# MoseleyBioinformaticsLab/ICIKendallTau

Hardware: AMD Instinct MI355X
Metric: column-pairs/s (+ full-matrix wall time) at 10k feat x 1k samp (higher is better)
Workload: dtype int32 rank/popcount counting + f64 epilogue

## Files before the change

icikendalltau_amd/csrc/icikt_capi.cpp:

```cpp
#include <hip/hip_runtime.h>

#include <algorithm>
#include <chrono>
#include <cstdio>
#include <cstring>
#include <functional>
#include <new>
#include <string>
#include <vector>

#include "icikt.h"
#include "icikt_device.h"
#include "icikt_host.h"

using icikt::ColStats;
using icikt::PairRaw;
using icikt::PrepView;

static_assert(ICIKT_CNT_FIELDS == icikt::ICIKT_CNT_FIELDS_, "counts record layout");
static_assert(ICIKT_PERSPECTIVE_LOCAL == icikt::ICIKT_PERSPECTIVE_LOCAL_, "perspective code");

namespace {

int flush_timer(icikt_ctx* c, int k) {
// ... 1486 lines not shown
                                      d_dst, dst_ld, c->d_csc_err.p, c->stream));
  unsigned long long rec[icikt::ICIKT_CSC_ERR_WORDS] = {};
  HIPCHK(c, hipMemcpyAsync(rec, c->d_csc_err.p, sizeof(rec), hipMemcpyDeviceToHost, c->stream));
  HIPCHK(c, hipStreamSynchronize(c->stream));
  if (rec[0] != 0) return fail(c, ICIKT_E_INVALID, "scatter_csc: " + icikt::host::csc_message(rec));
  return ICIKT_SUCCESS;
}

}

extern "C" {

int icikt_debug_set_plan(icikt_ctx* c, const char* spec) {
  if (!c) return ICIKT_E_INVALID;
  icikt_ctx::PlanOverride ov;
  int pipe = -1, k0 = -1;
  std::string sp = spec ? spec : "";
  size_t pos = 0;
  while (pos < sp.size()) {
    size_t end = sp.find(',', pos);
    if (end == std::string::npos) end = sp.size();
    const std::string item = sp.substr(pos, end - pos);
    pos = end + 1;
    if (item.empty()) continue;
    const size_t eq = item.find('=');
    if (eq == std::string::npos) return fail(c, ICIKT_E_INVALID, "debug_set_plan: expected key=value, got '" + item + "'");
    const std::string key = item.substr(0, eq), val = item.substr(eq + 1);
    if (val.empty()) continue;
    if (key == "np") ov.np = atoi(val.c_str());
    else if (key == "pend") ov.pend = (val[0] == 'g') ? 1 : 0;
    else if (key == "wpb") ov.wpb = atoi(val.c_str());
    else if (key == "half") ov.half = (val[0] == '1') ? 1 : 0;
    else if (key == "hyb") ov.hyb = (val[0] == '1') ? 1 : 0;
    else if (key == "tgmax") { ov.has_tgmax = true; ov.tgmax = atoi(val.c_str()); }
    else if (key == "list") ov.list = atoi(val.c_str());
    else if (key == "solo") ov.solo = atoi(val.c_str());
    else if (key == "split") ov.split = atoi(val.c_str());
    else if (key == "merge") ov.merge = atoi(val.c_str());
    else if (key == "waves") ov.waves = atoi(val.c_str());
    else if (key == "verbose") ov.verbose = (val[0] == '1');
    else if (key == "gridmult") ov.grid_mult = atoi(val.c_str());
    else if (key == "gridcap") ov.grid_cap = atoi(val.c_str());
    else if (key == "pipe") pipe = (val[0] == '1') ? 1 : 0;
    else if (key == "k0") k0 = (val[0] == '1') ? 1 : 0;
    else if (key == "tkblock") ov.tkblock = atoll(val.c_str());
    else if (key == "medlds") {
      ov.medlds = atoi(val.c_str());
      if (ov.medlds < 0 || ov.medlds > icikt::MEDIAN_STAGE_MAX)
        return fail(c, ICIKT_E_INVALID, "debug_set_plan: medlds must be in 0 .. 4096 keys");
    }
    else if (key == "qbatch") {
      ov.qbatch = atoi(val.c_str());
      if (ov.qbatch < 1 || ov.qbatch > icikt::QUANT_BATCH_MAX)
        return fail(c, ICIKT_E_INVALID, "debug_set_plan: qbatch must be in 1 .. 32 targets");
    }
    else return fail(c, ICIKT_E_INVALID, "debug_set_plan: unknown key '" + key + "'");
  }
  c->plan_ov = ov;
  c->pipe_mode = pipe;
  c->k0_shape = k0;

  c->raw_valid = false;
  c->wpb = 0;
  return ICIKT_SUCCESS;
}

int icikt_debug_step_stats(icikt_ctx* c, uint64_t* out24, int reset) {
  if (!c || !out24) return ICIKT_E_INVALID;
  int rc = use_device(c);
  if (rc) return rc;
  HIPCHK(c, hipStreamSynchronize(c->stream));
  unsigned long long tmp[24];
  const hipError_t e = icikt::read_step_stats(tmp, reset);
  if (e == hipErrorNotSupported) { (void)hipGetLastError(); return fail(c, ICIKT_E_STATE, "debug_step_stats: not a -DICIKT_STEP_STATS build"); }
  HIPCHK(c, e);
  for (int i = 0; i < 24; ++i) out24[i] = tmp[i];
  return ICIKT_SUCCESS;
}

int icikt_selftest(icikt_ctx* c) {
  if (!c) return ICIKT_E_INVALID;
  int rc = use_device(c);
  if (rc) return rc;
  HIPCHK(c, c->d_self.reserve(640));
  HIPCHK(c, icikt::launch_selftest(c->d_self.p, c->stream));
  uint32_t h[640];
  HIPCHK(c, hipMemcpyAsync(h, c->d_self.p, sizeof(h), hipMemcpyDeviceToHost, c->stream));
  HIPCHK(c, hipStreamSynchronize(c->stream));
  for (uint32_t l = 0; l < 64; ++l) {
    if (h[l] != (l + 1) * (l + 2) / 2) return fail(c, ICIKT_E_HIP, "selftest: wave_incl_scan mismatch");
    if (h[64 + l] != (l == 0 ? 0xABCDu : 3u * (l - 1))) return fail(c, ICIKT_E_HIP, "selftest: wave_shr1 mismatch");
    if (h[128 + l] != (l < 41 ? 0xFFFFFFFFu : l - 41)) return fail(c, ICIKT_E_HIP, "selftest: repeated wave_shr1 mismatch");
    if (h[256 + l] != (l < 32 ? l : 100u + (l - 32))) return fail(c, ICIKT_E_HIP, "selftest: permlane32_swap[0] mismatch");
    if (h[320 + l] != (l < 32 ? 32u + l : 100u + l)) return fail(c, ICIKT_E_HIP, "selftest: permlane32_swap[1] mismatch");
    const uint32_t k = (l & 31u) + 1, b = (l & 32u) + 1;
    if (h[384 + l] != k * (2 * b + k - 1) / 2) return fail(c, ICIKT_E_HIP, "selftest: half_incl_scan mismatch");
    if (h[448 + l] != 63u) {
      if (c->plan_ov.verbose) fprintf(stderr, "[icikt] selftest lane %u: lane_xor pass mask %u\n", l, h[448 + l]);
      return fail(c, ICIKT_E_HIP, "selftest: lane_xor mismatch");
    }
  }
  for (uint32_t half = 0; half < 2; ++half) {
    uint32_t want = 0, got = 0;
    for (uint32_t l = half * 32; l < half * 32 + 32; ++l) {
      const uint32_t lo = ((l * 40503u + 977u) >> 3) & 0xFFFu;
      for (uint32_t j = half * 32; j < l; ++j) want += (((j * 2654435761u >> 20) & 0xFFFu) < lo) ? 1u : 0u;
      got += h[192 + l];
    }
    if (got != want) {
      if (c->plan_ov.verbose) fprintf(stderr, "[icikt] selftest half %u: got %u want %u\n", half, got, want);
      return fail(c, ICIKT_E_HIP, "selftest: half_allpairs mismatch");
    }
  }
  for (uint32_t half = 0; half < 2; ++half) {
    uint32_t want = 0, got = 0;
    for (uint32_t l = half * 32; l < half * 32 + 32; ++l) {
      const uint32_t lo = ((l * 40503u + 977u) >> 3) & 0xFFFu, lo2 = ((l * 69069u + 12345u) >> 5) & 0x27BFu;
      for (uint32_t j = half * 32; j < l; ++j) {
        want += (((j * 2654435761u >> 20) & 0xFFFu) < lo) ? 1u : 0u;
        want += (((j * 1103515245u >> 17) & 0x27BFu) < lo2) ? 1u : 0u;
      }
      got += h[576 + l];
    }
    if (got != want) {
      if (c->plan_ov.verbose) fprintf(stderr, "[icikt] selftest half %u (packed): got %u want %u\n", half, got, want);
      return fail(c, ICIKT_E_HIP, "selftest: half_step_count mismatch");
    }
  }
  return ICIKT_SUCCESS;
}

}
```

icikendalltau_amd/csrc/icikt_kernels.hip:

```cpp
#include <hip/hip_runtime.h>
#include <stdint.h>
#include <stdlib.h>

#include <algorithm>
#include <type_traits>

#include "icikt_device.h"
#include "icikt_wave.h"

namespace icikt {

struct WaveLds {
  unsigned long long* seen;
  uint16_t* spre;
};

#define ICIKT_HSHR(b) "v_sub_co_u32_dpp %1, vcc, %2, %3 row_shr:" #b " row_mask:0xf bank_mask:0xf bound_ctrl:0\n\t" \
                      "v_addc_co_u32_e32 %0, vcc, 0, %0, vcc\n\t"
#define ICIKT_HROR(b) "v_sub_co_u32_dpp %1, vcc, %4, %5 row_ror:" #b " row_mask:0xf bank_mask:0xf\n\t" \
                      "v_addc_co_u32_e32 %0, vcc, 0, %0, vcc\n\t"
__device__ __forceinline__ uint32_t half_allpairs(uint32_t q, uint32_t lo, uint32_t xa, uint32_t xb, uint32_t lane) {
  uint32_t acc = 0, junk;
  asm volatile("s_nop 1\n\t"
               ICIKT_HSHR(1) ICIKT_HSHR(2) ICIKT_HSHR(3) ICIKT_HSHR(4) ICIKT_HSHR(5) ICIKT_HSHR(6) ICIKT_HSHR(7)
// ... 13 lines not shown
  const uint32_t rot = (uint32_t)__builtin_amdgcn_update_dpp(0, (int)r[1], 0x121 , 0xf, 0xf, false);
  const uint32_t xa = (lane & 16u) ? r[0] : rot;
  return half_allpairs(q, lo, xa, ~offer, lane);
}

#define ICIKT_PACC  "v_perm_b32 %1, %1, %2, %6\n\tv_lshrrev_b32_e32 %0, 1, %0\n\tv_and_or_b32 %0, %1, %5, %0\n\t"
#define ICIKT_PSHR2(a, b) "v_add_u32_dpp %1, %3, %4 row_shr:" #a " row_mask:0xf bank_mask:0xf bound_ctrl:0\n\t" \
                          "v_add_u32_dpp %2, %3, %4 row_shr:" #b " row_mask:0xf bank_mask:0xf bound_ctrl:0\n\t" ICIKT_PACC
#define ICIKT_PROR2(a, b) "v_add_u32_dpp %1, %3, %4 row_ror:" #a " row_mask:0xf bank_mask:0xf\n\t" \
                          "v_add_u32_dpp %2, %3, %4 row_ror:" #b " row_mask:0xf bank_mask:0xf\n\t" ICIKT_PACC
__device__ __forceinline__ uint32_t half_partner_addr(uint32_t lane) {
  const uint32_t p = lane & 15u, h = lane & 32u;
  return ((lane & 16u) ? (h + p) : (h + 16u + ((p + 15u) & 15u))) * 4u;
}
struct HalfChain { uint32_t A, B, offer, xa; };
__device__ __forceinline__ HalfChain half_step_prep(uint32_t sw0, uint32_t sw1, uint32_t lane, uint32_t partner_addr) {
  HalfChain h;
  const uint32_t Q = __builtin_amdgcn_perm(sw1, sw0, 0x05040100u);
  const uint32_t LO = __builtin_amdgcn_perm(sw1, sw0, 0x07060302u);
  h.A = 0x7FFF7FFFu - Q; h.B = LO;
  h.offer = (lane & 16u) ? h.B : h.A;
  h.xa = (uint32_t)__builtin_amdgcn_ds_bpermute((int)partner_addr, (int)h.offer);
  return h;
}
__device__ __forceinline__ uint32_t half_step_part_a(const HalfChain& h, uint32_t acc) {
  const uint32_t A = h.A, B = h.B, xa = h.xa, offer = h.offer;
  const uint32_t M8 = 0x80808080u, SEL = 0x07050301u;
  uint32_t v1, t1, t2;
  asm volatile("s_nop 1\n\t"
               "v_add_u32_dpp %1, %3, %4 row_shr:1 row_mask:0xf bank_mask:0xf bound_ctrl:0\n\t"
               "v_add_u32_dpp %2, %3, %4 row_shr:2 row_mask:0xf bank_mask:0xf bound_ctrl:0\n\t"
               "v_perm_b32 %1, %1, %2, %6\n\tv_and_b32_e32 %0, %5, %1\n\t"
               ICIKT_PSHR2(3, 4) ICIKT_PSHR2(5, 6) ICIKT_PSHR2(7, 8) ICIKT_PSHR2(9, 10) ICIKT_PSHR2(11, 12)
               ICIKT_PSHR2(13, 14)
               "v_add_u32_dpp %1, %3, %4 row_shr:15 row_mask:0xf bank_mask:0xf bound_ctrl:0\n\t"
               "v_add_u32_e32 %2, %7, %8\n\t" ICIKT_PACC
               : "=&v"(v1), "=&v"(t1), "=&v"(t2)
               : "v"(A), "v"(B), "s"(M8), "s"(SEL), "v"(xa), "v"(offer));
  return bcnt_acc(v1, acc);
}
__device__ __forceinline__ uint32_t half_step_part_b(const HalfChain& h, uint32_t acc) {
  const uint32_t xa = h.xa, offer = h.offer;
  const uint32_t M8 = 0x80808080u, SEL = 0x07050301u, M16 = 0x80008000u;
  uint32_t v2, t1, t2;
  asm volatile("s_nop 1\n\t"
               "v_add_u32_dpp %1, %3, %4 row_ror:1 row_mask:0xf bank_mask:0xf\n\t"
               "v_add_u32_dpp %2, %3, %4 row_ror:2 row_mask:0xf bank_mask:0xf\n\t"
               "v_perm_b32 %1, %1, %2, %6\n\tv_and_b32_e32 %0, %5, %1\n\t"
               ICIKT_PROR2(3, 4) ICIKT_PROR2(5, 6)
               "v_add_u32_dpp %1, %3, %4 row_ror:7 row_mask:0xf bank_mask:0xf\n\t"
               "v_lshrrev_b32_e32 %0, 1, %0\n\tv_and_or_b32 %0, %1, %7, %0\n\t"
               : "=&v"(v2), "=&v"(t1), "=&v"(t2)
               : "v"(xa), "v"(offer), "s"(M8), "s"(SEL), "s"(M16));
  return bcnt_acc(v2, acc);
}
__device__ __forceinline__ uint32_t half_step_count(uint32_t sw0, uint32_t sw1, uint32_t lane, uint32_t partner_addr) {
  const uint32_t Q = __builtin_amdgcn_perm(sw1, sw0, 0x05040100u);
  const uint32_t LO = __builtin_amdgcn_perm(sw1, sw0, 0x07060302u);
  const uint32_t A = 0x7FFF7FFFu - Q, B = LO;
  const uint32_t offer = (lane & 16u) ? B : A;
  const uint32_t xa = (uint32_t)__builtin_amdgcn_ds_bpermute((int)partner_addr, (int)offer);
  const uint32_t M8 = 0x80808080u, SEL = 0x07050301u, M16 = 0x80008000u;
  uint32_t v1, v2, t1, t2;
  asm volatile("s_nop 1\n\t"
               "v_add_u32_dpp %1, %3, %4 row_shr:1 row_mask:0xf bank_mask:0xf bound_ctrl:0\n\t"
               "v_add_u32_dpp %2, %3, %4 row_shr:2 row_mask:0xf bank_mask:0xf bound_ctrl:0\n\t"
               "v_perm_b32 %1, %1, %2, %6\n\tv_and_b32_e32 %0, %5, %1\n\t"
               ICIKT_PSHR2(3, 4) ICIKT_PSHR2(5, 6) ICIKT_PSHR2(7, 8) ICIKT_PSHR2(9, 10) ICIKT_PSHR2(11, 12)
               ICIKT_PSHR2(13, 14)
               "v_add_u32_dpp %1, %3, %4 row_shr:15 row_mask:0xf bank_mask:0xf bound_ctrl:0\n\t"
               "v_add_u32_e32 %2, %7, %8\n\t" ICIKT_PACC
               : "=&v"(v1), "=&v"(t1), "=&v"(t2)
               : "v"(A), "v"(B), "s"(M8), "s"(SEL), "v"(xa), "v"(offer));
  asm volatile("s_nop 1\n\t"
               "v_add_u32_dpp %1, %3, %4 row_ror:1 row_mask:0xf bank_mask:0xf\n\t"
               "v_add_u32_dpp %2, %3, %4 row_ror:2 row_mask:0xf bank_mask:0xf\n\t"
               "v_perm_b32 %1, %1, %2, %6\n\tv_and_b32_e32 %0, %5, %1\n\t"
               ICIKT_PROR2(3, 4) ICIKT_PROR2(5, 6)
               "v_add_u32_dpp %1, %3, %4 row_ror:7 row_mask:0xf bank_mask:0xf\n\t"
               "v_lshrrev_b32_e32 %0, 1, %0\n\tv_and_or_b32 %0, %1, %7, %0\n\t"
               : "=&v"(v2), "=&v"(t1), "=&v"(t2)
               : "v"(xa), "v"(offer), "s"(M8), "s"(SEL), "s"(M16));
  return bcnt_acc(v2, bcnt_acc(v1, 0u));
}

__device__ __forceinline__ void half_step_flags(uint32_t src, uint32_t own, uint32_t offer, uint32_t partner_addr,
                                                uint32_t& v1, uint32_t& v2) {
  const uint32_t xa = (uint32_t)__builtin_amdgcn_ds_bpermute((int)partner_addr, (int)offer);
  const uint32_t M8 = 0x80808080u, SEL = 0x07050301u, M16 = 0x80008000u;
  uint32_t t1, t2;
  asm volatile("s_nop 1\n\t"
               "v_add_u32_dpp %1, %3, %4 row_shr:1 row_mask:0xf bank_mask:0xf bound_ctrl:0\n\t"
               "v_add_u32_dpp %2, %3, %4 row_shr:2 row_mask:0xf bank_mask:0xf bound_ctrl:0\n\t"
               "v_perm_b32 %1, %1, %2, %6\n\tv_and_b32_e32 %0, %5, %1\n\t"
               ICIKT_PSHR2(3, 4) ICIKT_PSHR2(5, 6) ICIKT_PSHR2(7, 8) ICIKT_PSHR2(9, 10) ICIKT_PSHR2(11, 12)
               ICIKT_PSHR2(13, 14)
               "v_add_u32_dpp %1, %3, %4 row_shr:15 row_mask:0xf bank_mask:0xf bound_ctrl:0\n\t"
               "v_add_u32_e32 %2, %7, %8\n\t" ICIKT_PACC
               : "=&v"(v1), "=&v"(t1), "=&v"(t2)
               : "v"(src), "v"(own), "s"(M8), "s"(SEL), "v"(xa), "v"(offer));
  asm volatile("s_nop 1\n\t"
               "v_add_u32_dpp %1, %3, %4 row_ror:1 row_mask:0xf bank_mask:0xf\n\t"
               "v_add_u32_dpp %2, %3, %4 row_ror:2 row_mask:0xf bank_mask:0xf\n\t"
               "v_perm_b32 %1, %1, %2, %6\n\tv_and_b32_e32 %0, %5, %1\n\t"
               ICIKT_PROR2(3, 4) ICIKT_PROR2(5, 6)
               "v_add_u32_dpp %1, %3, %4 row_ror:7 row_mask:0xf bank_mask:0xf\n\t"
               "v_lshrrev_b32_e32 %0, 1, %0\n\tv_and_or_b32 %0, %1, %7, %0\n\t"
               : "=&v"(v2), "=&v"(t1), "=&v"(t2)
               : "v"(xa), "v"(offer), "s"(M8), "s"(SEL), "s"(M16));
}

template <int C>
__device__ __forceinline__ void half_step_flags_near(uint32_t src, uint32_t own, uint32_t offer, uint32_t partner_addr,
                                                     uint32_t& v1, uint32_t& v2) {
  const uint32_t xa = (uint32_t)__builtin_amdgcn_ds_bpermute((int)partner_addr, (int)offer);
  const uint32_t M8 = 0x80808080u, SEL = 0x07050301u, M16 = 0x80008000u;
  uint32_t t1, t2;
#define ICIKT_NEAR_HEAD "s_nop 1\n\t"                                                                          \
               "v_add_u32_dpp %1, %3, %4 row_shr:1 row_mask:0xf bank_mask:0xf bound_ctrl:0\n\t"                \
               "v_add_u32_dpp %2, %3, %4 row_shr:2 row_mask:0xf bank_mask:0xf bound_ctrl:0\n\t"                \
               "v_perm_b32 %1, %1, %2, %6\n\tv_and_b32_e32 %0, %5, %1\n\t"
  if constexpr (C == 0) {
    asm volatile(ICIKT_NEAR_HEAD "v_lshrrev_b32_e32 %0, 7, %0\n\t"
                 : "=&v"(v1), "=&v"(t1), "=&v"(t2) : "v"(src), "v"(own), "s"(M8), "s"(SEL));
  } else if constexpr (C == 1) {
    asm volatile(ICIKT_NEAR_HEAD ICIKT_PSHR2(3, 4) "v_lshrrev_b32_e32 %0, 6, %0\n\t"
                 : "=&v"(v1), "=&v"(t1), "=&v"(t2) : "v"(src), "v"(own), "s"(M8), "s"(SEL));
  } else {
    asm volatile(ICIKT_NEAR_HEAD ICIKT_PSHR2(3, 4) ICIKT_PSHR2(5, 6) ICIKT_PSHR2(7, 8) "v_lshrrev_b32_e32 %0, 4, %0\n\t"
                 : "=&v"(v1), "=&v"(t1), "=&v"(t2) : "v"(src), "v"(own), "s"(M8), "s"(SEL));
  }
#undef ICIKT_NEAR_HEAD
#define ICIKT_NEAR_HEAD2 "s_nop 1\n\t"                                                                         \
               "v_add_u32_dpp %1, %3, %4 row_ror:1 row_mask:0xf bank_mask:0xf\n\t"                             \
               "v_add_u32_dpp %2, %3, %4 row_ror:2 row_mask:0xf bank_mask:0xf\n\t"                             \
               "v_perm_b32 %1, %1, %2, %6\n\tv_and_b32_e32 %0, %5, %1\n\t"
  if constexpr (C == 0) {
    asm volatile(ICIKT_NEAR_HEAD2 "v_lshrrev_b32_e32 %0, 3, %0\n\t"
                 : "=&v"(v2), "=&v"(t1), "=&v"(t2) : "v"(xa), "v"(offer), "s"(M8), "s"(SEL));
  } else if constexpr (C == 1) {
    asm volatile(ICIKT_NEAR_HEAD2 ICIKT_PROR2(3, 4) "v_lshrrev_b32_e32 %0, 2, %0\n\t"
                 : "=&v"(v2), "=&v"(t1), "=&v"(t2) : "v"(xa), "v"(offer), "s"(M8), "s"(SEL));
  } else {
    asm volatile(ICIKT_NEAR_HEAD2 ICIKT_PROR2(3, 4) ICIKT_PROR2(5, 6)
                 "v_add_u32_dpp %1, %3, %4 row_ror:7 row_mask:0xf bank_mask:0xf\n\t"
                 "v_lshrrev_b32_e32 %0, 1, %0\n\tv_and_or_b32 %0, %1, %7, %0\n\t"
                 : "=&v"(v2), "=&v"(t1), "=&v"(t2) : "v"(xa), "v"(offer), "s"(M8), "s"(SEL), "s"(M16));
  }
#undef ICIKT_NEAR_HEAD2
}

__device__ __forceinline__ uint32_t wave_cross_idx(uint32_t lane, uint32_t c) {
  const uint32_t later = (c == 1u) ? (lane & 16u) : (lane & 32u);
  const uint32_t prow = (lane ^ (c << 4)) & 48u;
  return (prow | ((later ? lane : lane - 1u) & 15u)) << 2;
}
#define ICIKT_WROR(b, xa, xb) "v_sub_co_u32_dpp %1, vcc, " xa ", " xb " row_ror:" #b " row_mask:0xf bank_mask:0xf\n\t" \
                              "v_addc_co_u32_e32 %0, vcc, 0, %0, vcc\n\t"
#define ICIKT_WROUND(xa, xb)                                                                  \
  "v_cmp_lt_u32_e32 vcc, " xa ", " xb "\n\tv_addc_co_u32_e32 %0, vcc, 0, %0, vcc\n\t"        \
  ICIKT_WROR(1, xa, xb) ICIKT_WROR(2, xa, xb) ICIKT_WROR(3, xa, xb) ICIKT_WROR(4, xa, xb)     \
  ICIKT_WROR(5, xa, xb) ICIKT_WROR(6, xa, xb) ICIKT_WROR(7, xa, xb)
__device__ __forceinline__ uint32_t wave_allpairs(uint32_t q, uint32_t lo, uint32_t lane) {
  const uint32_t nlo = ~lo;
  const uint32_t off1 = (lane & 16u) ? nlo : q;
  const uint32_t off2 = (lane & 32u) ? nlo : q;
// ... 343 lines not shown
    my_ctr = task_ctr + xg;
    int t = 0;
    if (lane == 0u) t = atomicAdd(my_ctr, 1);
    task = t_lo + __builtin_amdgcn_readfirstlane(t);
  }
  const int split = half_mode_of<NP, HI>() ? k1_opt_segments(opts) : 1;
  int seg = 0;
  if (split > 1) {
    seg = gwave / n_tasks;
    task = gwave - seg * n_tasks;
    if (seg >= split) return;
  }
  if (task >= t_hi) return;
  do {
  ICIKT_ST_DECL
  int pidx[NP];
  pidx[0] = __builtin_amdgcn_readfirstlane(tasks[2 * task]);
  const int p_second = __builtin_amdgcn_readfirstlane(tasks[2 * task + 1]);
  const int np = (NP == 2 && p_second >= 0) ? 2 : 1;
  if (NP == 2) pidx[NP - 1] = (p_second >= 0) ? p_second : pidx[0];

  const int scol = __builtin_amdgcn_readfirstlane(pj[pidx[0]]);
  const uint16_t* ord = pv.order + (int64_t)scol * pv.n_ord;
  const uint32_t* ord_w = pv.order_w ? pv.order_w + (int64_t)scol * pv.n_ord : nullptr;
  const unsigned long long* gf = pv.col_gflag(scol);
  const unsigned long long* ma = pv.col_mask(scol);
  const unsigned long long* fa = pv.col_fillmask(scol);

  uint32_t comp[NP];
  const uint16_t* hiG[NP];
  const uint32_t* tgB[NP];
  int ntgB[NP];
  bool cntB[NP];
  PairState S[NP];
  uint32_t cb[NP], gg[NP];
  bool g_oddtie = false;
  const uint32_t* rec_blk;
  const uint32_t* hi_blk;
  const uint32_t* gi_blk;
  {
    const int g0 = __builtin_amdgcn_readfirstlane(pi[pidx[0]]);
    rec_blk = pv.rec + ((int64_t)(g0 >> 1) * pv.rec_rows) * 2;
    hi_blk = reinterpret_cast<const uint32_t*>(pv.hirow + ((int64_t)(g0 >> 1) * pv.rec_rows) * 2);
    gi_blk = reinterpret_cast<const uint32_t*>(pv.girow + ((int64_t)(g0 >> 1) * pv.rec_rows) * 2);
  }
#pragma unroll
  for (int k = 0; k < NP; ++k) {
    const int gcol = __builtin_amdgcn_readfirstlane(pi[pidx[k]]);
    comp[k] = (uint32_t)(gcol & 1);
    hiG[k] = pv.hirow + ((int64_t)(gcol >> 1) * pv.rec_rows) * 2 + (gcol & 1);
    tgB[k] = pv.tgroups + (int64_t)gcol * pv.tg_stride;
    const int ntg_raw = __builtin_amdgcn_readfirstlane((int)pv.col_stats(gcol)->ntg);
    cntB[k] = half_mode ? (ntg_raw > tg_list) : (ntg_raw > max(tg_list, K1_CNT_MIN_GROUPS));
    ntgB[k] = (!(opts & K1_OPT_ROW_ONLY) && ntg_raw <= ((half_mode || cntB[k]) ? max(tg_list, tg_max) : tg_list)) ? ntg_raw : -1;
    g_oddtie = g_oddtie || (__builtin_amdgcn_readfirstlane(pv.col_stats(gcol)->flags) & COL_ODD_TIE) != 0;
    const unsigned long long* mb = pv.col_mask(gcol);
    const unsigned long long* fb = pv.col_fillmask(gcol);

    unsigned char* wbase = smem + ((size_t)wave * NP + k) * (size_t)perpair_bytes;
    S[k].L.seen = reinterpret_cast<unsigned long long*>(wbase);
    if (HI == 0) {
      S[k].L.spre = reinterpret_cast<uint16_t*>(S[k].L.seen + Wp4);
      for (int w = lane; w < Wp4; w += 64) S[k].L.seen[w] = 0ull;
      uint32_t* tl32 = reinterpret_cast<uint32_t*>(S[k].L.spre);
      for (int w = lane; w < (TL_BYTES + (cnt_cap > 0 ? (cnt_cap + 2) * ICIKT_CNT_BYTES + 3 : 0)) / 4; w += 64) tl32[w] = 0u;
    } else {
      S[k].L.spre = reinterpret_cast<uint16_t*>(S[k].L.seen + Wp4);
      for (int w = lane; w < Wp4; w += 64) S[k].L.seen[w] = 0ull;
      for (int w = lane; w < k1_half_pre_bytes<(HI > 0 ? HI : 1)>() / 2; w += 64) S[k].L.spre[w] = 0;
      uint32_t* cz = reinterpret_cast<uint32_t*>(reinterpret_cast<unsigned char*>(S[k].L.spre) + k1_half_pre_bytes<(HI > 0 ? HI : 1)>());
      for (int w = lane; w < ((tg_max + 2) * ICIKT_CNT_BYTES + 3) / 4; w += 64) cz[w] = 0u;
    }
    S[k].dis = 0; S[k].tie = 0; S[k].tie2 = 0;
    cb[k] = 0; gg[k] = 0;
    if (seg == 0) {
      for (int w = lane; w < W; w += 64) {
        cb[k] += (uint32_t)__popcll(ma[w] & mb[w]);
        gg[k] += (uint32_t)__popcll(fa[w] & fb[w]);
      }
    }
  }
  wave_lds_fence();

  uint32_t r0 = gload_u16(ord, lane), r1 = gload_u16(ord, 64u + lane), r2 = gload_u16(ord, 128u + lane);
  uint32_t rk_pre[NP];
  uint2 rv_pre = make_uint2(0u, 0u);
  bool rk_ok = false;
#pragma unroll
  for (int k = 0; k < NP; ++k) rk_pre[k] = 0u;
  uint32_t hi_pre = 0;
  uint32_t gi_pre = 0;
  bool hi_ok = false;

  const uint32_t solo_cap = (uint32_t)max(0, (tg_max + 1) * ICIKT_CNT_BYTES);
  bool solo_ok = half_mode && !(opts & K1_OPT_ROW_ONLY) && !(opts & K1_OPT_NO_SOLO);
#pragma unroll
  for (int k = 0; k < NP; ++k) solo_ok = solo_ok && (pv.col_stats(__builtin_amdgcn_readfirstlane(pi[pidx[k]]))->ntg <= solo_cap);
  int last_start;
  bool closed_form = true;
#pragma unroll
  for (int k = 0; k < NP; ++k) closed_form = closed_form && (ntgB[k] >= 0);
  int hot_until;
  {
    int best = 0, first_cont = n;
    for (int w = lane; w < W; w += 64) {
      unsigned long long f = gf[w];
      unsigned long long z = ~f;
      if (w == W - 1 && (n & 63)) { f &= (1ull << (n & 63)) - 1ull; z &= (1ull << (n & 63)) - 1ull; }
      if (f != 0ull) best = max(best, w * 64 + 63 - (int)__builtin_clzll(f));
      if (z != 0ull) first_cont = min(first_cont, w * 64 + (int)__builtin_ctzll(z));
    }
    last_start = __builtin_amdgcn_readfirstlane(wave_max_i32(best));
    first_cont = -__builtin_amdgcn_readfirstlane(wave_max_i32(-first_cont));
    hot_until = (first_cont < n) ? first_cont - 1 : n;
    closed_form = closed_form && (n - last_start > 64);
  }
  int seg_begin = 0, seg_end = n, seg_step = -1;
  if constexpr (half_mode) {
    if (split > 1) {
      const uint32_t* tail = pv.tprog + (int64_t)scol * pv.tp_stride + (pv.tp_stride - 2 * TPROG_MARKS);
      const uint32_t mv = gload_u32(tail, lane & 7u);
      auto mark = [&](int j, int& mp, int& ms) {
        mp = (int)min((uint32_t)__builtin_amdgcn_readlane((int)mv, j), (uint32_t)n);
        ms = __builtin_amdgcn_readlane((int)mv, 4 + j);
      };
      int b1 = n, b2 = n, b3 = n, s1 = -1, s2 = -1, s3 = -1;
      if (split == 2) mark(1, b1, s1);
      else { mark(0, b1, s1); mark(2, b2, s2); mark(3, b3, s3); }
      seg_begin = (seg == 0) ? 0 : (seg == 1) ? b1 : (seg == 2) ? b2 : b3;
      seg_end = (seg == 0) ? b1 : (seg == 1) ? b2 : (seg == 2) ? b3 : n;
      seg_step = (seg == 0) ? -1 : (seg == 1) ? s1 : (seg == 2) ? s2 : s3;
      if (seg > 0 && seg_begin >= seg_end) return;
      closed_form = closed_form && (seg_end >= n);
      hot_until = min(hot_until, seg_end);
    }
  }
  const int end_main = min(closed_form ? last_start : n, seg_end);

  const uint32_t partner_addr = half_partner_addr(lane);
  uint32_t dis_half = 0, dis_half_neg = 0;
  uint32_t seg_tie = 0, seg_tie2 = 0;
  bool grp_open = false;
  int grp_start = 0, grp_entries = 0;
  uint32_t sv_k0 = 0, sv_k1 = 0, sv_h = 0;
  uint32_t sv_kw[NP], sv_hw[NP], sv_gw[NP], sneg[NP];
#pragma unroll
  for (int k = 0; k < NP; ++k) { sv_kw[k] = 0u; sv_hw[k] = 0u; sv_gw[k] = 0u; sneg[k] = 0u; }
  int pos = 0;
  if constexpr (half_mode) {
    if (seg_begin > 0) {
      constexpr int HP = (HI > 0 ? HI : 1);
      const bool hiP = lane >= 32u;
      const uint32_t l32p = lane & 31u;
      unsigned long long* seenP = hiP ? S[NP - 1].L.seen : S[0].L.seen;
      uint16_t* spreP = hiP ? S[NP - 1].L.spre : S[0].L.spre;
      const uint32_t GUARDP = (uint32_t)W << 6;
      const uint32_t ord_last = (uint32_t)pv.n_ord - 1u;
      uint32_t rw[4];
#pragma unroll
      for (int u = 0; u < 4; ++u) rw[u] = gload_u16(ord, min((uint32_t)u * 64u + lane, ord_last));
      for (int p = 0; p < seg_begin; p += 256) {
        uint2 rv[4];
#pragma unroll
        for (int u = 0; u < 4; ++u) rv[u] = gload_rec2(rec_blk, rw[u]);
#pragma unroll
        for (int u = 0; u < 4; ++u) rw[u] = gload_u16(ord, min((uint32_t)p + 256u + (uint32_t)u * 64u + lane, ord_last));
#pragma unroll
        for (int u = 0; u < 4; ++u) {
          const int pu = p + 64 * u;
          const auto sw = __builtin_amdgcn_permlane32_swap(comp[0] ? rv[u].y : rv[u].x, comp[NP - 1] ? rv[u].y : rv[u].x, false, false);
          const bool w0 = pu + (int)l32p < seg_begin, w1 = pu + 32 + (int)l32p < seg_begin;
          seen_insert(seenP, w0 ? (sw[0] & 0xFFFFu) : GUARDP);
          seen_insert(seenP, w1 ? (sw[1] & 0xFFFFu) : GUARDP);
        }
      }
      wave_lds_fence();
      rebuild_prefix_half<HP>(seenP, spreP, l32p);
      wave_lds_fence();
      pos = seg_begin;
      r0 = gload_u16(ord, (uint32_t)pos + lane);
      r1 = gload_u16(ord, (uint32_t)pos + 64u + lane);
      r2 = gload_u16(ord, (uint32_t)pos + 128u + lane);
    }
  }
  ICIKT_ST_MARK(6, 0)
  unsigned long long fw0 = 0ull, fw1 = 0ull;
  int fw_word = -1;
  const uint32_t* tprog_col = half_mode ? pv.tprog + (int64_t)scol * pv.tp_stride : nullptr;
  const uint16_t* srow_col = half_mode ? pv.srow + (int64_t)scol * pv.sr_steps * 64 : nullptr;
  const uint2* smask_col = half_mode ? pv.smask + (int64_t)scol * pv.sr_steps * 32 : nullptr;
  uint32_t tp_a = 0u, tp_b = 0u;
  int tp_step = 0;
  bool tp_ok = false;
  auto advance64 = [&]() {
    r0 = r1; r1 = r2;
    if (NP == 2) rv_pre = gload_rec2(rec_blk, r0);
    else rk_pre[0] = gload_u32(rec_blk, 2u * r0 + comp[0]);
    r2 = gload_u16(ord, (uint32_t)pos + 128u + lane);
    rk_ok = true;
  };
  auto take_rk = [&](uint32_t (&rk)[NP]) {
    if (NP == 2) {
#pragma unroll
      for (int k = 0; k < NP; ++k) rk[k] = comp[k] ? rv_pre.y : rv_pre.x;
    } else {
      rk[0] = rk_pre[0];
    }
  };
  bool defer_allpairs = false;
  uint32_t mix_sg1 = 0u, mix_sg2 = 0u;
  int mix_cls = 3;
  uint32_t solo_g0 = 0u, solo_g1 = 0u;
  auto hot_step = [&](const uint32_t (&rk)[NP], auto mode_tag) {
    constexpr int MODE = decltype(mode_tag)::value;
    constexpr bool MIXED = MODE == 1;
    if constexpr (half_mode) {
      const auto sw = __builtin_amdgcn_permlane32_swap(rk[0], rk[NP - 1], false, false);
      const bool hi = lane >= 32u;
      unsigned long long* seenH = hi ? S[NP - 1].L.seen : S[0].L.seen;
      uint16_t* spreH = hi ? S[NP - 1].L.spre : S[0].L.spre;
      const uint32_t l32 = lane & 31u;
      constexpr int H = (HI > 0 ? HI : 1);
      uint32_t inpairs = 0;
#pragma unroll
      for (int sub = 0; sub < 2; ++sub) {
        const uint32_t r = sub ? sw[1] : sw[0];
        const uint32_t qh = r & 0xFFFFu, loh = r >> 16;
        const uint32_t wlo = r >> 22;
        const uint32_t dlo = (wlo * (65536u / (uint32_t)H + 1u)) >> 16;
        const uint32_t pre_lo = (uint32_t)*reinterpret_cast<const uint16_t*>(
            reinterpret_cast<const unsigned char*>(spreH) + 2u * wlo + (2u * (uint32_t)k1_half_slot<H>() - 2u * (uint32_t)H) * dlo);
        const unsigned long long word_lo = seenH[wlo];
        wave_lds_fence();
        atomicOr(reinterpret_cast<uint32_t*>(seenH) + __builtin_amdgcn_ubfe(r, 5, 10), 1u << (qh & 31u));
        wave_lds_fence();
        unsigned long long wv[H];
#pragma unroll
        for (int i = 0; i < H; ++i) wv[i] = seenH[l32 * (uint32_t)H + (uint32_t)i];
        uint32_t solo_c = 1u;
        uint8_t* cntS = nullptr;
        if constexpr (MODE == 2) {
          const uint32_t g = sub ? solo_g1 : solo_g0;
          cntS = reinterpret_cast<uint8_t*>(spreH) + k1_half_pre_bytes<H>();
          if (g < solo_cap) atomicAdd(reinterpret_cast<uint32_t*>(cntS) + (g >> 2), 1u << ((g & 3u) << 3));
          wave_lds_fence();
          solo_c = (g < solo_cap) ? (uint32_t)cntS[g] : 1u;
        }
        if (sub == 0 && MODE != 2) {
          if constexpr (!MIXED) {
            inpairs = half_step_count(sw[0], sw[1], lane, partner_addr);
          } else {
            const uint32_t Q = __builtin_amdgcn_perm(sw[1], sw[0], 0x05040100u);
            const uint32_t LO = __builtin_amdgcn_perm(sw[1], sw[0], 0x07060302u);
            const uint32_t A = 0x7FFF7FFFu - Q, B = LO;
            uint32_t f1, f2, g1, g2;
            half_step_flags(A, B, (lane & 16u) ? B : A, partner_addr, f1, f2);
            if (mix_cls == 0) half_step_flags_near<0>(B, A, (lane & 16u) ? A : B, partner_addr, g1, g2);
            else if (mix_cls == 1) half_step_flags_near<1>(B, A, (lane & 16u) ? A : B, partner_addr, g1, g2);
            else if (mix_cls == 2) half_step_flags_near<2>(B, A, (lane & 16u) ? A : B, partner_addr, g1, g2);
            else half_step_flags(B, A, (lane & 16u) ? A : B, partner_addr, g1, g2);
            inpairs = bcnt_acc(f2 & ~mix_sg2, bcnt_acc(f1 & ~mix_sg1, 0u));
            seg_tie = bcnt_acc(mix_sg2 & ~(f2 | g2), bcnt_acc(mix_sg1 & ~(f1 | g1), seg_tie));
          }
        }
        uint32_t pre_lo_k = pre_lo;
        unsigned long long word_lo_k = word_lo;
        asm volatile("" : "+v"(pre_lo_k), "+v"(word_lo_k));
#pragma unroll
        for (int i = 0; i < H; ++i) asm volatile("" : "+v"(wv[i]));
        dis_half += pre_lo_k + (sub == 0 ? inpairs : 0u);
        dis_half_neg = bcnt64_acc(word_lo_k >> (loh & 63u), dis_half_neg);
        uint32_t cw[H], run = 0;
#pragma unroll
        for (int i = 0; i < H; ++i) {
          run = bcnt64_acc(wv[i], run);
          cw[i] = run;
        }
        half_pre_store<H>(spreH, l32, half_incl_scan(run), cw);
        if constexpr (MODE == 2) {
          const uint32_t g = sub ? solo_g1 : solo_g0;
          seg_tie2 += solo_c - 1u;
          wave_lds_fence();
          if (g < solo_cap) cntS[g] = 0;
        }
        wave_lds_fence();
      }
    } else {
      TwoLevel T[NP];
#pragma unroll
      for (int k = 0; k < NP; ++k) {
        T[k] = tl_view(S[k].L.seen, S[k].L.spre);
        S[k].dis += tl_query(T[k], rk[k] >> 16, IT, magic);
      }
      if (!defer_allpairs) {
#pragma unroll
        for (int k = 0; k < NP; ++k) S[k].dis += wave_allpairs(rk[k] & 0xFFFFu, rk[k] >> 16, lane);
      }
      wave_lds_fence();
      if constexpr (NP == 1) {
        seen_insert(S[0].L.seen, rk[0] & 0xFFFFu);
        tl_update(T[0], true, rk[0] & 0xFFFFu, IT, magic, lane);
      } else {
#pragma unroll
        for (int k = 0; k < NP; ++k) {
          const uint32_t qk = rk[k] & 0xFFFFu;
          seen_insert(S[k].L.seen, qk);
          tl_update_rows(T[k], qk);
        }
        wave_lds_fence();
        uint32_t hh[NP];
#pragma unroll
        for (int k = 0; k < NP; ++k) hh[k] = atomicExch(&T[k].hist[lane], 0u);
#pragma unroll
        for (int k = 0; k < NP; ++k) {
          const uint32_t below = wave_incl_scan(hh[k]) - hh[k];
          if (below != 0u) atomicAdd(&T[k].lb[lane], below);
        }
      }
      wave_lds_fence();
    }
  };
  while (pos < end_main) {
    if (pos + 64 <= hot_until) {
      const bool halved = (HI == 0) && (n > 32768) && !g_oddtie;
      const bool pack2 = (HI == 0) && ((n <= 32768) || halved);
      uint32_t rk_prev[NP];
#pragma unroll
      for (int k = 0; k < NP; ++k) rk_prev[k] = 0u;
      if (NP == 2 && HI == 0 && pack2 && (opts & K1_OPT_HALF_LAYOUT)) {
        const bool hiH = lane >= 32u;
        const uint32_t l32 = lane & 31u;
        const TwoLevel TH = tl_view(hiH ? S[NP - 1].L.seen : S[0].L.seen, hiH ? S[NP - 1].L.spre : S[0].L.spre);
        unsigned long long* const hist2 = reinterpret_cast<unsigned long long*>(TH.hist) + l32;
        unsigned long long* const lb2 = reinterpret_cast<unsigned long long*>(TH.lb) + l32;
        uint32_t dh = 0u;
        do {
          uint32_t rk[NP];
          if (rk_ok) {
            take_rk(rk);
          } else {
            const uint2 rv = gload_rec2(rec_blk, r0);
#pragma unroll
            for (int k = 0; k < NP; ++k) rk[k] = comp[k] ? rv.y : rv.x;
          }
          pos += 64;
          advance64();
          const auto sw = __builtin_amdgcn_permlane32_swap(rk[0], rk[NP - 1], false, false);
          HalfChain hc;
          {
            uint32_t ka = sw[0], kb = sw[1];
            if (halved) {
              ka = (((ka + 0x10000u) >> 1) & 0x7FFF0000u) | ((ka >> 1) & 0x7FFFu);
              kb = (((kb + 0x10000u) >> 1) & 0x7FFF0000u) | ((kb >> 1) & 0x7FFFu);
            }
            hc = half_step_prep(ka, kb, lane, partner_addr);
          }
#pragma unroll
          for (int sub = 0; sub < 2; ++sub) {
            const uint32_t r = sub ? sw[1] : sw[0];
            const uint32_t cnt = tl_query(TH, r >> 16, IT, magic);
            wave_lds_fence();
            seen_insert(TH.seen, r & 0xFFFFu);
            tl_update_rows(TH, r & 0xFFFFu);
            wave_lds_fence();
            const unsigned long long hh = atomicExch(hist2, 0ull);
            if (sub == 0) dh = half_step_part_a(hc, dh);
            else dh = half_step_part_b(hc, dh);
            dh += cnt;
            const uint32_t h0 = (uint32_t)hh, h1 = (uint32_t)(hh >> 32), hs = h0 + h1;
            const uint32_t below0 = half_incl_scan(hs) - hs, below1 = below0 + h0;
            if ((below0 | below1) != 0u) atomicAdd(lb2, (unsigned long long)below0 | ((unsigned long long)below1 << 32));
            wave_lds_fence();
          }
          ICIKT_ST_MARK(0, 64)
        } while (pos + 64 <= hot_until);
        S[0].dis += hiH ? 0u : dh;
        S[NP - 1].dis += hiH ? dh : 0u;
      } else
      if (HI == 0 && pack2) {
        int ph[NP];
#pragma unroll
        for (int k = 0; k < NP; ++k) ph[k] = (k == 0) ? 1 : 0;
        do {
          uint32_t rk[NP];
          if (rk_ok) {
            take_rk(rk);
          } else if (NP == 2) {
            const uint2 rv = gload_rec2(rec_blk, r0);
#pragma unroll
            for (int k = 0; k < NP; ++k) rk[k] = comp[k] ? rv.y : rv.x;
          } else {
            rk[0] = gload_u32(rec_blk, 2u * r0 + comp[0]);
          }
          pos += 64;
          advance64();
          TwoLevel T[NP];
          uint32_t cnt[NP];
#pragma unroll
          for (int k = 0; k < NP; ++k) {
            T[k] = tl_view(S[k].L.seen, S[k].L.spre);
            cnt[k] = tl_query(T[k], rk[k] >> 16, IT, magic);
          }
          Packed2 pk[NP];
#pragma unroll
          for (int k = 0; k < NP; ++k) {
            if (ph[k] == 2) {
              uint32_t ka = rk_prev[k], kb = rk[k];
              if (halved) {
                ka = (((ka + 0x10000u) >> 1) & 0x7FFF0000u) | ((ka >> 1) & 0x7FFFu);
                kb = (((kb + 0x10000u) >> 1) & 0x7FFF0000u) | ((kb >> 1) & 0x7FFFu);
              }
              pk[k] = wave_allpairs_packed2_prep(ka, kb, lane);
            }
          }
#pragma unroll
          for (int k = 0; k < NP; ++k) {
            S[k].dis += cnt[k];
            if (ph[k] == 0) S[k].dis += wave_allpairs(rk[k] & 0xFFFFu, rk[k] >> 16, lane);
          }
          wave_lds_fence();
#pragma unroll
          for (int k = 0; k < NP; ++k) {
            seen_insert(S[k].L.seen, rk[k] & 0xFFFFu);
            tl_update_rows(T[k], rk[k] & 0xFFFFu);
          }
          wave_lds_fence();
          uint32_t hh[NP];
#pragma unroll
          for (int k = 0; k < NP; ++k) hh[k] = atomicExch(&T[k].hist[lane], 0u);
#pragma unroll
          for (int k = 0; k < NP; ++k)
            if (ph[k] == 2) S[k].dis += wave_allpairs_packed2_count(pk[k]);
#pragma unroll
          for (int k = 0; k < NP; ++k) {
            const uint32_t below = wave_incl_scan(hh[k]) - hh[k];
            if (below != 0u) atomicAdd(&T[k].lb[lane], below);
          }
          wave_lds_fence();
#pragma unroll
          for (int k = 0; k < NP; ++k) {
            if (ph[k] == 1) { rk_prev[k] = rk[k]; ph[k] = 2; }
            else ph[k] = 1;
          }
          ICIKT_ST_MARK(0, 64)
        } while (pos + 64 <= hot_until);
#pragma unroll
        for (int k = 0; k < NP; ++k)
          if (ph[k] == 2) S[k].dis += wave_allpairs(rk_prev[k] & 0xFFFFu, rk_prev[k] >> 16, lane);
      } else {
      do {
        uint32_t rk[NP];
        if (rk_ok) {
          take_rk(rk);
        } else if (NP == 2) {
          const uint2 rv = gload_rec2(rec_blk, r0);
#pragma unroll
          for (int k = 0; k < NP; ++k) rk[k] = comp[k] ? rv.y : rv.x;
        } else {
          rk[0] = gload_u32(rec_blk, 2u * r0 + comp[0]);
        }
        pos += 64;
        advance64();
        hot_step(rk, std::integral_constant<int, 0>{});
        ICIKT_ST_MARK(0, 64)
      } while (pos + 64 <= hot_until);
      }
      defer_allpairs = false;
      hi_ok = false;
      continue;
    }
    if constexpr (half_mode) {
      if (!tp_ok) {
        const int tp_base = (seg_step > 0) ? seg_step : 0;
        uint32_t off = (uint32_t)tp_base;
        asm volatile("" : "+v"(off));
        tp_a = gload_u32(tprog_col, off);
        tp_b = gload_u32(tprog_col, off + 1u);
        r0 = gload_u16(srow_col, (uint32_t)tp_base * 64u + lane);
        r1 = gload_u16(srow_col, (uint32_t)tp_base * 64u + 64u + lane);
        r2 = gload_u16(srow_col, (uint32_t)tp_base * 64u + 128u + lane);
        rv_pre = gload_rec2(rec_blk, r0);
        tp_step = tp_base;
        tp_ok = true;
        rk_ok = true;
        hi_ok = false;
      }
    }
    const uint32_t row = r0;
    const uint32_t hi_now = hi_pre;
    const uint32_t gi_now = gi_pre;
    const bool hi_now_ok = hi_ok;
    uint32_t rk[NP];
    if (rk_ok) {
      take_rk(rk);
    } else if (NP == 2) {
      const uint2 rv = gload_rec2(rec_blk, row);
#pragma unroll
      for (int k = 0; k < NP; ++k) rk[k] = comp[k] ? rv.y : rv.x;
    } else {
      rk[0] = gload_u32(rec_blk, 2u * row + comp[0]);
    }
    int nact;
    bool Fn;
    unsigned long long F;
    int kind = 0;
    bool closes = true;
    uint32_t e_next = 0u;
    uint2 tmx = make_uint2(0u, 0u);
    if constexpr (half_mode) {
      const uint32_t e = (uint32_t)__builtin_amdgcn_readfirstlane((int)tp_a);
      e_next = (uint32_t)__builtin_amdgcn_readfirstlane((int)tp_b);
      tp_a = tp_b;
      {
        uint32_t off = (uint32_t)(tp_step + 2);
        asm volatile("" : "+v"(off));
        tp_b = gload_u32(tprog_col, off);
      }
      nact = (int)tprog_rows(e);
      kind = (int)tprog_kind(e);
      closes = tprog_closes(e);
      Fn = (kind == 2) ? closes : true;
      F = (kind == 0) ? ~0ull : 0ull;
      if (kind == 3) kind = solo_ok ? 3 : 1;
      if (kind == 1) {
        tmx = smask_col[(uint32_t)tp_step * 32u + (lane & 31u)];
        mix_cls = (int)((e >> 16) & 3u);
      }
    } else
    if (pos + 64 <= hot_until) {
      nact = 64; Fn = true; F = ~0ull;
    } else {
      const int wc = pos >> 6, fb = pos & 63;
      if (fw_word != wc) {
        fw0 = gf[min(wc, W)];
        fw1 = gf[min(wc + 1, W)];
        fw_word = wc;
      }
      const unsigned long long w0 = uniform_u64(fw0), w1 = uniform_u64(fw1);
      F = fb ? ((w0 >> fb) | (w1 << (64 - fb))) : w0;
      const bool fnbit = ((w1 >> fb) & 1ull) != 0ull;
      const int remaining = end_main - pos;
      const bool reach_end = remaining <= 64;
      if (remaining < 64) F &= (1ull << remaining) - 1ull;
      {
        constexpr int SW = half_mode ? 32 : 64;
        const int avail = reach_end ? remaining : 64;
// ... 718 lines not shown
            const uint32_t row = ordB[k];
            const uint32_t lo = loA[row], hi = hiA[row];
            const uint32_t cell = wide_query(pend, ppre, hi + 1u) - wide_query(pend, ppre, lo);
            tie2 += cell - 1u;
          }
        }
        wave_lds_fence();
        for (int w = (int)lane; w < Wp; w += 64) { seen[w] |= pend[w]; pend[w] = 0ull; }
        wave_lds_fence();
        wide_rebuild(seen, pre, Wp, lane);
        wave_lds_fence();
        pos = gend;
        continue;
      }
      int nact;
      if (end_at_64) nact = 64;
      else nact = 63 - (int)__builtin_clzll(starts);
      const bool valid = (int)lane < nact;
      uint32_t q = 0xFFFFFFFFu, lo = 0u;
      if (valid) {
        const uint32_t row = ordB[pos + (int)lane];
        q = qA[row];
        lo = loA[row];
      }
      const uint32_t gid = (uint32_t)__popcll(F & ((2ull << lane) - 1ull));
      if (valid) dis += wide_query(seen, pre, lo);
      uint32_t sq = q, sg = gid, slo = lo;
      if (nact == 64 && F == ~0ull) {
        dis += wave_allpairs(q, lo, lane);
      } else
      for (int d = 1; d < nact; ++d) {
        sq = dpp_wave_shr1(0xFFFFFFFFu, sq);
        sg = dpp_wave_shr1(0xFFFFFFFFu, sg);
        slo = dpp_wave_shr1(0xFFFFFFFFu, slo);
        if (valid && (int)lane >= d) {
          if (sg != gid) dis += (sq < lo) ? 1u : 0u;
          else tie += (slo == lo) ? 1u : 0u;
        }
      }
      wave_lds_fence();
      if (valid) seen_insert(seen, q);
      wave_lds_fence();
      wide_rebuild(seen, pre, Wp, lane);
      wave_lds_fence();
      pos += nact;
    }
    const unsigned long long* ma = pv.col_mask(ca);
    const unsigned long long* mb = pv.col_mask(cb_);
    const unsigned long long* fa = pv.col_fillmask(ca);
    const unsigned long long* fbm = pv.col_fillmask(cb_);
    unsigned long long cboth = 0, gboth = 0;
    for (int w = (int)lane; w < W; w += 64) {
      cboth += (unsigned long long)__popcll(ma[w] & mb[w]);
      gboth += (unsigned long long)__popcll(fa[w] & fbm[w]);
    }
    const unsigned long long dis_t = wave_sum_u64(dis);
    const unsigned long long tie_t = wave_sum_u64(tie) + (wave_sum_u64(tie2) >> 1);
    const unsigned long long cb_t = wave_sum_u64(cboth), gg_t = wave_sum_u64(gboth);
    if (lane == 0u) {
      PairRaw o;
      o.dis = dis_t;
      o.ntie = tie_t;
      o.c_both = (uint32_t)cb_t;
      o.g = (uint32_t)gg_t;
      raw[p] = o;
    }
    wave_lds_fence();
  }
}

__global__ void k_selftest(uint32_t* out) {
  const uint32_t lane = lane_id();
  out[lane] = wave_incl_scan(lane + 1u);
  out[64 + lane] = dpp_wave_shr1(0xABCDu, lane * 3u);
  uint32_t v = dpp_wave_shr1(0xFFFFFFFFu, lane);
  for (int s = 1; s < 41; ++s) v = dpp_wave_shr1(v, v);
  out[128 + lane] = v;
  const uint32_t q = (lane * 2654435761u >> 20) & 0xFFFu, lo = ((lane * 40503u + 977u) >> 3) & 0xFFFu;
  out[192 + lane] = half_count(q, lo, lane);
  {
    const uint32_t q2 = (lane * 1103515245u >> 17) & 0x27BFu, lo2 = ((lane * 69069u + 12345u) >> 5) & 0x27BFu;
    out[576 + lane] = half_step_count(q | (lo << 16), q2 | (lo2 << 16), lane, half_partner_addr(lane));
  }
  const auto sw = __builtin_amdgcn_permlane32_swap(lane, 100u + lane, false, false);
  out[256 + lane] = sw[0];
  out[320 + lane] = sw[1];
  out[384 + lane] = half_incl_scan(lane + 1u);
  const uint32_t t5 = lane * 5u + 1u;
  out[448 + lane] = (lane_xor<1>(t5, lane) == ((lane ^ 1u) * 5u + 1u) ? 1u : 0u) |
                    (lane_xor<2>(t5, lane) == ((lane ^ 2u) * 5u + 1u) ? 2u : 0u) |
                    (lane_xor<4>(t5, lane) == ((lane ^ 4u) * 5u + 1u) ? 4u : 0u) |
                    (lane_xor<8>(t5, lane) == ((lane ^ 8u) * 5u + 1u) ? 8u : 0u) |
                    (lane_xor<16>(t5, lane) == ((lane ^ 16u) * 5u + 1u) ? 16u : 0u) |
                    (lane_xor<32>(t5, lane) == ((lane ^ 32u) * 5u + 1u) ? 32u : 0u);
  out[512 + lane] = 0u;
}

hipError_t launch_k1_wide(const PrepView& pv, const int32_t* pi, const int32_t* pj, PairRaw* raw, int64_t n_pairs,
                          int blocks, size_t lds_bytes, int* task_ctr, hipStream_t s) {
  if (n_pairs <= 0 || blocks <= 0) return hipSuccess;
  (void)hipGetLastError();
  hipError_t e = hipFuncSetAttribute(reinterpret_cast<const void*>(k1_wide), hipFuncAttributeMaxDynamicSharedMemorySize,
                                     (int)lds_bytes);
  if (e != hipSuccess) return e;
  hipLaunchKernelGGL(k1_wide, dim3(blocks), dim3(64), lds_bytes, s, pv, pi, pj, raw, (long long)n_pairs, task_ctr);
  return hipGetLastError();
}
hipError_t k1_wide_blocks_per_cu(size_t lds_bytes, int* out) {
  hipError_t e = hipFuncSetAttribute(reinterpret_cast<const void*>(k1_wide), hipFuncAttributeMaxDynamicSharedMemorySize,
                                     (int)lds_bytes);
  if (e != hipSuccess) return e;
  return hipOccupancyMaxActiveBlocksPerMultiprocessor(out, reinterpret_cast<const void*>(k1_wide), 64, lds_bytes);
}

__global__ void __launch_bounds__(256) k_zero_raw(const int32_t* __restrict__ tasks, int n_tasks, PairRaw* __restrict__ raw) {
  const int t = (int)(blockIdx.x * 256 + threadIdx.x);
  if (t >= n_tasks) return;
  PairRaw z;
  z.dis = 0ull; z.ntie = 0ull; z.c_both = 0u; z.g = 0u;
  const int p0 = tasks[2 * t], p1 = tasks[2 * t + 1];
  raw[p0] = z;
  if (p1 >= 0) raw[p1] = z;
}
hipError_t launch_zero_raw(const int32_t* tasks, int n_tasks, PairRaw* raw, hipStream_t s) {
  if (n_tasks <= 0) return hipSuccess;
  (void)hipGetLastError();
  hipLaunchKernelGGL(k_zero_raw, dim3((n_tasks + 255) / 256), dim3(256), 0, s, tasks, n_tasks, raw);
  return hipGetLastError();
}

typedef void (*k1_fn_t)(PrepView, const int32_t*, int, const int32_t*, const int32_t*, PairRaw*, int, int*, int);

static k1_fn_t k1_select(int np, int half_items) {
  if (np == 2) {
    switch (half_items) {
      case 0: return &k1_pairs<2, 0>;
      case 1: return &k1_pairs<2, 1>;
      case 2: return &k1_pairs<2, 2>;
      case 3: return &k1_pairs<2, 3>;
      case 4: return &k1_pairs<2, 4>;
      case 5: return &k1_pairs<2, 5>;
      case 6: return &k1_pairs<2, 6>;
      case 7: return &k1_pairs<2, 7>;
      case 9: return &k1_pairs<2, 9>;
      case 11: return &k1_pairs<2, 11>;
      case 13: return &k1_pairs<2, 13>;
      case 15: return &k1_pairs<2, 15>;
      default: return nullptr;
    }
  }
  if (np != 1 || half_items != 0) return nullptr;
  return &k1_pairs<1, 0>;
}

hipError_t launch_k1(const PrepView& pv, const int32_t* tasks, int n_tasks, const int32_t* pi,
                     const int32_t* pj, PairRaw* raw, int np, int half_items, int wpb, int blocks,
                     size_t lds_bytes, int perpair_bytes, int* task_ctr, int opts, hipStream_t s) {
  if (n_tasks <= 0 || blocks <= 0) return hipSuccess;
  k1_fn_t fn = k1_select(np, half_items);
  if (!fn) return hipErrorInvalidValue;
  (void)hipGetLastError();
  hipError_t e = hipFuncSetAttribute(reinterpret_cast<const void*>(fn), hipFuncAttributeMaxDynamicSharedMemorySize,
                                     (int)lds_bytes);
  if (e != hipSuccess) return e;
  hipLaunchKernelGGL(fn, dim3(blocks), dim3(wpb * 64), lds_bytes, s, pv, tasks, n_tasks, pi, pj, raw,
                     perpair_bytes, task_ctr, opts);
// ... 34 lines not shown
```

Measured before the change: 52.79 million.

## Use bit-reversed lane order in half-mode hot loop to drop row_shr DPP chain

Loads row order indices with bit-reversed lane indices within each 16-lane row in half mode. A new half_step_count_brev counts the within-half pairs using only row_ror DPP rotations plus lane-parity masks (cndmask with alternating bit patterns), replacing the shift-with-bound_ctrl sequence in the hot path. The aim is fewer DPP/ALU instructions per 64-element step. It adds a selftest entry for the new counting routine. The lane_ld reassignment at hot-loop entry and the MODE==3 dispatch must stay consistent with the other paths that load from ord.

Measured after the change: 53.30 million (median of 6 runs). No clear change (+1.0%).

```diff
diff --git a/icikendalltau_amd/csrc/icikt_capi.cpp b/icikendalltau_amd/csrc/icikt_capi.cpp
--- a/icikendalltau_amd/csrc/icikt_capi.cpp
+++ b/icikendalltau_amd/csrc/icikt_capi.cpp
@@ -1592,9 +1592,9 @@
   if (!c) return ICIKT_E_INVALID;
   int rc = use_device(c);
   if (rc) return rc;
-  HIPCHK(c, c->d_self.reserve(640));
+  HIPCHK(c, c->d_self.reserve(704));
   HIPCHK(c, icikt::launch_selftest(c->d_self.p, c->stream));
-  uint32_t h[640];
+  uint32_t h[704];
   HIPCHK(c, hipMemcpyAsync(h, c->d_self.p, sizeof(h), hipMemcpyDeviceToHost, c->stream));
   HIPCHK(c, hipStreamSynchronize(c->stream));
   for (uint32_t l = 0; l < 64; ++l) {
@@ -1623,7 +1623,7 @@
     }
   }
   for (uint32_t half = 0; half < 2; ++half) {
-    uint32_t want = 0, got = 0;
+    uint32_t want = 0, got = 0, got_brev = 0;
     for (uint32_t l = half * 32; l < half * 32 + 32; ++l) {
       const uint32_t lo = ((l * 40503u + 977u) >> 3) & 0xFFFu, lo2 = ((l * 69069u + 12345u) >> 5) & 0x27BFu;
       for (uint32_t j = half * 32; j < l; ++j) {
@@ -1631,13 +1631,18 @@
         want += (((j * 1103515245u >> 17) & 0x27BFu) < lo2) ? 1u : 0u;
       }
       got += h[576 + l];
+      got_brev += h[640 + l];
     }
     if (got != want) {
       if (c->plan_ov.verbose) fprintf(stderr, "[icikt] selftest half %u (packed): got %u want %u\n", half, got, want);
       return fail(c, ICIKT_E_HIP, "selftest: half_step_count mismatch");
     }
-  }
-  return ICIKT_SUCCESS;
-}
-
-}
+    if (got_brev != want) {
+      if (c->plan_ov.verbose) fprintf(stderr, "[icikt] selftest half %u (packed, bit-reversed): got %u want %u\n", half, got_brev, want);
+      return fail(c, ICIKT_E_HIP, "selftest: half_step_count_brev mismatch");
+    }
+  }
+  return ICIKT_SUCCESS;
+}
+
+}
diff --git a/icikendalltau_amd/csrc/icikt_kernels.hip b/icikendalltau_amd/csrc/icikt_kernels.hip
--- a/icikendalltau_amd/csrc/icikt_kernels.hip
+++ b/icikendalltau_amd/csrc/icikt_kernels.hip
@@ -119,6 +119,37 @@
                : "=&v"(v2), "=&v"(t1), "=&v"(t2)
                : "v"(xa), "v"(offer), "s"(M8), "s"(SEL), "s"(M16));
   return bcnt_acc(v2, bcnt_acc(v1, 0u));
+}
+
+__device__ __forceinline__ uint32_t half_brev_lane(uint32_t lane) {
+  return (lane & 48u) | (__builtin_bitreverse32(lane & 15u) >> 28);
+}
+#define ICIKT_BROR2(a, b) "v_add_u32_dpp %1, %3, %3 row_ror:" #a " row_mask:0xf bank_mask:0xf\n\t" \
+                          "v_add_u32_dpp %2, %3, %3 row_ror:" #b " row_mask:0xf bank_mask:0xf\n\t"
+__device__ __forceinline__ uint32_t half_step_count_brev(uint32_t sw0, uint32_t sw1, uint32_t lane, uint32_t partner_addr) {
+  const uint32_t Q = __builtin_amdgcn_perm(sw1, sw0, 0x05040100u);
+  const uint32_t LO = __builtin_amdgcn_perm(sw1, sw0, 0x07060302u);
+  const uint32_t A = 0x7FFF7FFFu - Q, B = LO;
+  const uint32_t offer = (lane & 16u) ? B : A;
+  uint32_t x = (uint32_t)__builtin_amdgcn_ds_bpermute((int)partner_addr, (int)offer);
+  const uint32_t M8 = 0x80808080u, SEL = 0x07050301u;
+  const unsigned long long L0 = 0xAAAAAAAAAAAAAAAAull, L1 = 0xCCCCCCCCCCCCCCCCull, L2 = 0xF0F0F0F0F0F0F0F0ull;
+  uint32_t v1, t1, t2;
+  asm volatile("v_add_u32_e32 %1, %3, %4\n\ts_nop 0\n\t"
+               "v_add_u32_dpp %2, %3, %4 row_ror:1 row_mask:0xf bank_mask:0xf\n\t"
+               "v_perm_b32 %1, %1, %2, %6\n\tv_and_b32_e32 %0, %5, %1\n\t"
+               ICIKT_PROR2(2, 3) ICIKT_PROR2(4, 5)
+               "v_add_u32_dpp %1, %3, %4 row_ror:6 row_mask:0xf bank_mask:0xf\n\t"
+               "v_add_u32_dpp %2, %3, %4 row_ror:7 row_mask:0xf bank_mask:0xf\n\t"
+               "v_cndmask_b32_e64 %3, %7, %8, %9\n\t" ICIKT_PACC
+               ICIKT_BROR2(1, 3) ICIKT_PACC
+               ICIKT_BROR2(5, 7) "v_cndmask_b32_e64 %3, %7, %8, %10\n\t" ICIKT_PACC
+               ICIKT_BROR2(2, 6) "v_cndmask_b32_e64 %3, %7, %8, %11\n\t" ICIKT_PACC
+               "v_add_u32_dpp %1, %3, %3 row_ror:4 row_mask:0xf bank_mask:0xf\n\t"
+               "v_add_u32_dpp %2, %7, %8 row_shr:8 row_mask:0xf bank_mask:0xf bound_ctrl:0\n\t" ICIKT_PACC
+               : "=&v"(v1), "=&v"(t1), "=&v"(t2), "+v"(x)
+               : "v"(offer), "s"(M8), "s"(SEL), "v"(A), "v"(B), "s"(L0), "s"(L1), "s"(L2));
+  return bcnt_acc(v1, 0u);
 }
 
 __device__ __forceinline__ void half_step_flags(uint32_t src, uint32_t own, uint32_t offer, uint32_t partner_addr,
@@ -628,7 +659,8 @@
   }
   wave_lds_fence();
 
-  uint32_t r0 = gload_u16(ord, lane), r1 = gload_u16(ord, 64u + lane), r2 = gload_u16(ord, 128u + lane);
+  uint32_t lane_ld = half_mode ? half_brev_lane(lane) : lane;
+  uint32_t r0 = gload_u16(ord, lane_ld), r1 = gload_u16(ord, 64u + lane_ld), r2 = gload_u16(ord, 128u + lane_ld);
   uint32_t rk_pre[NP];
   uint2 rv_pre = make_uint2(0u, 0u);
   bool rk_ok = false;
@@ -724,9 +756,9 @@
       rebuild_prefix_half<HP>(seenP, spreP, l32p);
       wave_lds_fence();
       pos = seg_begin;
-      r0 = gload_u16(ord, (uint32_t)pos + lane);
-      r1 = gload_u16(ord, (uint32_t)pos + 64u + lane);
-      r2 = gload_u16(ord, (uint32_t)pos + 128u + lane);
+      r0 = gload_u16(ord, (uint32_t)pos + lane_ld);
+      r1 = gload_u16(ord, (uint32_t)pos + 64u + lane_ld);
+      r2 = gload_u16(ord, (uint32_t)pos + 128u + lane_ld);
     }
   }
   ICIKT_ST_MARK(6, 0)
@@ -742,7 +774,7 @@
     r0 = r1; r1 = r2;
     if (NP == 2) rv_pre = gload_rec2(rec_blk, r0);
     else rk_pre[0] = gload_u32(rec_blk, 2u * r0 + comp[0]);
-    r2 = gload_u16(ord, (uint32_t)pos + 128u + lane);
+    r2 = gload_u16(ord, (uint32_t)pos + 128u + lane_ld);
     rk_ok = true;
   };
   auto take_rk = [&](uint32_t (&rk)[NP]) {
@@ -794,7 +826,8 @@
         }
         if (sub == 0 && MODE != 2) {
           if constexpr (!MIXED) {
-            inpairs = half_step_count(sw[0], sw[1], lane, partner_addr);
+            if constexpr (MODE == 3) inpairs = half_step_count_brev(sw[0], sw[1], lane, partner_addr);
+            else inpairs = half_step_count(sw[0], sw[1], lane, partner_addr);
           } else {
             const uint32_t Q = __builtin_amdgcn_perm(sw[1], sw[0], 0x05040100u);
             const uint32_t LO = __builtin_amdgcn_perm(sw[1], sw[0], 0x07060302u);
@@ -868,6 +901,11 @@
   };
   while (pos < end_main) {
     if (pos + 64 <= hot_until) {
+      if constexpr (half_mode) {
+        uint32_t lane_e = lane;
+        asm volatile("" : "+v"(lane_e));
+        lane_ld = half_brev_lane(lane_e);
+      }
       const bool halved = (HI == 0) && (n > 32768) && !g_oddtie;
       const bool pack2 = (HI == 0) && ((n <= 32768) || halved);
       uint32_t rk_prev[NP];
@@ -1007,7 +1045,7 @@
         }
         pos += 64;
         advance64();
-        hot_step(rk, std::integral_constant<int, 0>{});
+        hot_step(rk, std::integral_constant<int, half_mode ? 3 : 0>{});
         ICIKT_ST_MARK(0, 64)
       } while (pos + 64 <= hot_until);
       }
@@ -1892,6 +1930,12 @@
     const uint32_t q2 = (lane * 1103515245u >> 17) & 0x27BFu, lo2 = ((lane * 69069u + 12345u) >> 5) & 0x27BFu;
     out[576 + lane] = half_step_count(q | (lo << 16), q2 | (lo2 << 16), lane, half_partner_addr(lane));
   }
+  {
+    const uint32_t w = half_brev_lane(lane);
+    const uint32_t qw = (w * 2654435761u >> 20) & 0xFFFu, low = ((w * 40503u + 977u) >> 3) & 0xFFFu;
+    const uint32_t qw2 = (w * 1103515245u >> 17) & 0x27BFu, low2 = ((w * 69069u + 12345u) >> 5) & 0x27BFu;
+    out[640 + lane] = half_step_count_brev(qw | (low << 16), qw2 | (low2 << 16), lane, half_partner_addr(lane));
+  }
   const auto sw = __builtin_amdgcn_permlane32_swap(lane, 100u + lane, false, false);
   out[256 + lane] = sw[0];
   out[320 + lane] = sw[1];
```
